# krullgit/3D-Object-Detection-for-autonomous-navigation

Measured on AMD Instinct MI355X. Metric: frames/sec (whole node) + p50 per-frame ms, 16k-pt pillars, higher is better.
Workload: dtype f32 (GEMMs on the 16-bit matrix pipe as split operands -- two float16 pieces per value, 3 products, fp32 accumulate: fp32-equivalent results, measured 1.5e-6 max from the fp32 oracle at this shape)

## Files before the change

3d-object-detection-for-autonomous-navigation_amd/csrc/backbone.hip:

```cpp
#include <stdio.h>
#include <stdlib.h>
#include <string.h>

#include "pp_common.h"

typedef float f32x16 __attribute__((ext_vector_type(16)));
#if PP_SPLIT_MODE == 0
typedef __bf16 bf16x8 __attribute__((ext_vector_type(8)));
#define PC_MFMA(A, B, C) __builtin_amdgcn_mfma_f32_32x32x16_bf16(A, B, C, 0, 0, 0)
#else
typedef _Float16 bf16x8 __attribute__((ext_vector_type(8)));
#define PC_MFMA(A, B, C) __builtin_amdgcn_mfma_f32_32x32x16_f16(A, B, C, 0, 0, 0)
#endif
#if PP_SPLIT_MODE == 0
#define PC_LO(PTR) (*reinterpret_cast<const bf16x8*>(PTR))
#else
#define PC_LO(PTR) (bf16x8{})
#endif
#if PP_SPLIT_MODE == 0
#define PC_PRODUCTS(ACC, XH, XM, XL, YH, YM, YL) \
    ACC = PC_MFMA(XL, YH, ACC); ACC = PC_MFMA(XH, YL, ACC); ACC = PC_MFMA(XM, YM, ACC); \
    ACC = PC_MFMA(XM, YH, ACC); ACC = PC_MFMA(XH, YM, ACC); ACC = PC_MFMA(XH, YH, ACC);
#elif PP_SPLIT_MODE == 1
#define PC_PRODUCTS(ACC, XH, XM, XL, YH, YM, YL) \
    ACC = PC_MFMA(XM, YH, ACC); ACC = PC_MFMA(XH, YM, ACC); ACC = PC_MFMA(XH, YH, ACC);
#else
#define PC_PRODUCTS(ACC, XH, XM, XL, YH, YM, YL) \
    ACC = PC_MFMA(XM, YM, ACC); ACC = PC_MFMA(XM, YH, ACC); ACC = PC_MFMA(XH, YM, ACC); ACC = PC_MFMA(XH, YH, ACC);
#endif
typedef unsigned u32x4 __attribute__((ext_vector_type(4)));

__device__ __forceinline__ float4 buf_load16(__amdgpu_buffer_rsrc_t r, unsigned voff, unsigned soff) {
    const u32x4 v = __builtin_amdgcn_raw_buffer_load_b128(r, voff, soff, 0);
    return make_float4(__uint_as_float(v.x), __uint_as_float(v.y), __uint_as_float(v.z), __uint_as_float(v.w));
}
__device__ __forceinline__ void buf_store16(float4 v, __amdgpu_buffer_rsrc_t r, unsigned voff, unsigned soff) {
    const u32x4 u = {__float_as_uint(v.x), __float_as_uint(v.y), __float_as_uint(v.z), __float_as_uint(v.w)};
    __builtin_amdgcn_raw_buffer_store_b128(u, r, voff, soff, 0);
}
__device__ __forceinline__ __amdgpu_buffer_rsrc_t make_rsrc(const void* base) {
    return __builtin_amdgcn_make_buffer_rsrc(const_cast<void*>(base), 0, 0x7ffffffe, 0x00020000);
}

#define PX_TILE 128

int g_num_cus = 256;

static bool split_precision() {
    static int dflt = -1;
    if (dflt < 0) {
        const char* e = getenv("PP_GEMM_PREC");
        dflt = (e && e[0] == 'f') ? 0 : 1;
    }
    return dflt == 1;
}
#define KC 32
#define LDS_STRIDE 36

struct GemmArgs {
    const float* in;
    const float* dw;
    const float* wt;
    const unsigned short* wt16;
    int n_total;
    const float* bias;
    float* out;
    float* head;
    const float* head_wt;
    const float* head_wt16;
    const float* head_bias;
    int head_mode;
    int M;
    int tile_lo;
    int in_h, in_w, cin;
    int px_h, px_w;
    int stride;
    int ld_out, co_off;
    int epi;
    int k, cout;
    const int* occ;
    int occ_nz;
    const unsigned long long* occbits;
    int occ_w64;
    float* cls_plane;
    int cls_col0, cls_ncol;
// ... 509 lines not shown
        const f16x2_t m = __builtin_convertvector(r1, f16x2_t);
        hi[j] = h.x; hi[j + 1] = h.y;
        mid[j] = m.x; mid[j + 1] = m.y;
    }
    lo = mid;
}
#endif

__device__ __forceinline__ void fast_divmod(int n, int d, float inv_d, int& q, int& r) {
    q = (int)((float)n * inv_d);
    r = n - q * d;
    if (r < 0) { --q; r += d; }
    if (r >= d) { ++q; r -= d; }
}

template <int NT, int S, int WPS, int PREC, int OCC = 0, int TR = 0>
__global__ __launch_bounds__(256, WPS) void k_sep_u(GemmArgs a, int ntiles) {
    static_assert(TR == 0 || (PREC == 1 && OCC == 0), "training forward: split-precision, dense input");
    constexpr bool PW = TR == 2;
    constexpr int NTAP = (TR == 1) ? 11 : 9;
    constexpr int KCH = 16, LSTR = KCH + 4, G = 4;
    constexpr int WW = S + 3;
    constexpr int NLD = PW ? 2 : 3 * WW;
    constexpr int SAW = 32 * LSTR;
    constexpr int SB = (PREC == 0) ? NT * LSTR : PP_NPIECE * NT * 8;
    constexpr int NB4 = (PREC == 0) ? (NT * G + 255) / 256 : (NT * 2 * PP_NPIECE + 255) / 256;
    constexpr int NTILES = NT / 32;
    constexpr int KQ = KCH / 8;
    __shared__ __attribute__((aligned(16))) float smem[8 * SAW + 2 * SB + (PW ? 0 : NTAP * 256) + (TR ? 8 * NT : 0)];
    const int tid = threadIdx.x, lane = tid & 63, wave = tid >> 6;
    float* const sAw = smem + wave * 2 * SAW;
    float* const sB = smem + 8 * SAW;
    float* const sDW = smem + 8 * SAW + 2 * SB;
    [[maybe_unused]] float* const sST = smem + 8 * SAW + 2 * SB + (PW ? 0 : NTAP * 256);

    const int xcd = blockIdx.x & 7, gl = blockIdx.x >> 3, GL = gridDim.x >> 3;
    const int nt_ = ntiles - a.tile_lo;
    const int tbase = a.tile_lo + (int)(((long long)xcd * nt_) >> 3), tend = a.tile_lo + (int)(((long long)(xcd + 1) * nt_) >> 3);
    const int first = tbase + gl;
    const int n0 = blockIdx.y * NT;
    if (first >= tend) {
        if (TR && a.tr_stat != nullptr && tid < 2 * NT)
            a.tr_stat[((size_t)blockIdx.x * 2 + tid / NT) * a.n_total + n0 + tid % NT] = 0.f;
        if (TR && a.tr_stat != nullptr && tid == 0 && blockIdx.y == 0) a.tr_stat[(size_t)gridDim.x * 2 * a.n_total + blockIdx.x] = 0.f;
        return;
    }
    const int ntl = (tend - first + GL - 1) / GL;
    const int cin = a.cin;
    const int nchunks = cin / KCH;
// ... 67 lines not shown
            aoff[e] = (ok_ ? rowoff_[dy_] + coloff_[dx_] : 0u) + (unsigned)(c4 * 16);                    \
        }                                                                                                \
        }                                                                                                \
    }
    constexpr int NBI = (PREC == 0) ? NT * G : NT * 2 * PP_NPIECE;
    unsigned boff[NB4];
    int bdst[NB4];
#pragma unroll
    for (int r = 0; r < NB4; ++r) {
        const int e_ = (tid + 256 * r) % NBI;
        if (PREC == 0) {
            boff[r] = (unsigned)(((n0 + e_ / G) * cin + (e_ % G) * 4) * 4);
            bdst[r] = (e_ / G) * LSTR + (e_ % G) * 4;
        } else {
            const int piece = e_ / (NT * 2), rem = e_ % (NT * 2), row = rem >> 1, half = rem & 1;
            boff[r] = (unsigned)(((piece * a.n_total + n0 + row) * 16 + half * 8) * 2);
            bdst[r] = piece * (NT * 8) + row * 8 + ((half ^ ((row >> 3) & 1)) * 4);
        }
    }
    const unsigned bstep = (PREC == 0) ? (unsigned)(KCH * 4) : (unsigned)(PP_NPIECE * a.n_total * 32);
    float4 rin[NLD];
    float4 rb0, rb1, rb2;
    rb0 = rb1 = rb2 = make_float4(0.f, 0.f, 0.f, 0.f);
    static_assert(NB4 <= 3, "weight prefetch registers");
#define U_LOAD_ACT(KCIDX, RIN)                                                                           \
    {                                                                                                    \
        const unsigned so_ = (unsigned)(KCIDX) * (KCH * 4);                                              \
        _Pragma("unroll") for (int e = 0; e < NLD; ++e) RIN[e] = buf_load16(rs_in, aoff[e], so_);        \
    }
#define U_LOAD_WT(KCIDX)                                                                                 \
    {                                                                                                    \
        const unsigned sb_ = (unsigned)(KCIDX) * bstep;                                                  \
// ... 4 lines not shown
#define U_LOAD_CHUNK(KCIDX) { U_LOAD_ACT(KCIDX, rin) U_LOAD_WT(KCIDX) }
    int ld_tile = first, ld_kc = 0;
    int st_kc = 0;
    int mm_tile = first, mm_kc = 0;
    [[maybe_unused]] float st_n = 0.f;
    U_TILE_OFFSETS(ld_tile)
    U_LOAD_CHUNK(0)
    ld_kc = 1;
    {
        const int ngrp = cin / 4;
        if (!PW) for (int e = tid; e < 9 * ngrp; e += 256) {
            const int t = e / ngrp, g4 = e - t * ngrp;
            reinterpret_cast<float4*>(sDW)[g4 * NTAP + t] = reinterpret_cast<const float4*>(a.dw)[e];
        }
        if (TR) for (int e = tid; e < 8 * NT; e += 256) sST[e] = 0.f;
        if (tr_act) {
            for (int g4 = tid; g4 < ngrp; g4 += 256) {
                const float4 q0 = a.tr_coef[4 * g4], q1 = a.tr_coef[4 * g4 + 1], q2 = a.tr_coef[4 * g4 + 2], q3 = a.tr_coef[4 * g4 + 3];
                reinterpret_cast<float4*>(sDW)[g4 * NTAP + 9] = make_float4(q0.x, q1.x, q2.x, q3.x);
                reinterpret_cast<float4*>(sDW)[g4 * NTAP + 10] = make_float4(q0.y, q1.y, q2.y, q3.y);
            }
        }
    }

    f32x16 acc[NTILES];
#pragma unroll
    for (int n = 0; n < NTILES; ++n)
#pragma unroll
        for (int r = 0; r < 16; ++r) acc[n][r] = 0.f;
    const int h = lane >> 5, r32 = lane & 31;
    float bias_r[NTILES];
#pragma unroll
    for (int n = 0; n < NTILES; ++n) bias_r[n] = (TR && a.bias == nullptr) ? 0.f : a.bias[n0 + n * 32 + r32];
    __syncthreads();

#define U_MFMA(I)                                                                                        \
    if (PREC == 1) {                                                                                     \
        const float* cA = cA0 + ((I) & 1) * SAW;                                                         \
        const float* cB = cB0 + ((I) & 1) * SB;                                                          \
        const float4 a0 = *reinterpret_cast<const float4*>(cA), a1 = *reinterpret_cast<const float4*>(cA + 4);  \
        const float av[8] = {a0.x, a0.y, a0.z, a0.w, a1.x, a1.y, a1.z, a1.w};                            \
        bf16x8 ah, am, al;                                                                               \
        split_bf16x3(av, ah, am, al);                                                                    \
        _Pragma("unroll") for (int n = 0; n < NTILES; ++n) {                                             \
            const bf16x8 bh = *reinterpret_cast<const bf16x8*>(cB + n * 32 * 8);                         \
            const bf16x8 bm = *reinterpret_cast<const bf16x8*>(cB + NT * 8 + n * 32 * 8);                \
            [[maybe_unused]] const bf16x8 bl = PC_LO(cB + 2 * NT * 8 + n * 32 * 8);            \
            PC_PRODUCTS(acc[n], ah, am, al, bh, bm, bl)                                                  \
        }                                                                                                \
    }                                                                                                    \
    if (PREC == 0) {                                                                                     \
        const float* cA = sAw + ((I) & 1) * SAW + r32 * LSTR + h * (KCH / 2);                            \
        const float* cB = sB + ((I) & 1) * SB + r32 * LSTR + h * (KCH / 2);                              \
        float4 a4[KQ];                                                                                   \
        _Pragma("unroll") for (int qq = 0; qq < KQ; ++qq) a4[qq] = *reinterpret_cast<const float4*>(cA + qq * 4);  \
        _Pragma("unroll") for (int n = 0; n < NTILES; ++n) {                                             \
            float4 b4[KQ];                                                                               \
            _Pragma("unroll") for (int qq = 0; qq < KQ; ++qq) b4[qq] = *reinterpret_cast<const float4*>(cB + n * 32 * LSTR + qq * 4);  \
            _Pragma("unroll") for (int qq = 0; qq < KQ; ++qq) {                                          \
                acc[n] = __builtin_amdgcn_mfma_f32_32x32x2f32(a4[qq].x, b4[qq].x, acc[n], 0, 0, 0);      \
                acc[n] = __builtin_amdgcn_mfma_f32_32x32x2f32(a4[qq].y, b4[qq].y, acc[n], 0, 0, 0);      \
                acc[n] = __builtin_amdgcn_mfma_f32_32x32x2f32(a4[qq].z, b4[qq].z, acc[n], 0, 0, 0);      \
                acc[n] = __builtin_amdgcn_mfma_f32_32x32x2f32(a4[qq].w, b4[qq].w, acc[n], 0, 0, 0);      \
// ... 21 lines not shown
                    o0.x = fmaf(v0.x, w4.x, o0.x); o0.y = fmaf(v0.y, w4.y, o0.y);                        \
                    o0.z = fmaf(v0.z, w4.z, o0.z); o0.w = fmaf(v0.w, w4.w, o0.w);                        \
                    o1.x = fmaf(v1.x, w4.x, o1.x); o1.y = fmaf(v1.y, w4.y, o1.y);                        \
                    o1.z = fmaf(v1.z, w4.z, o1.z); o1.w = fmaf(v1.w, w4.w, o1.w);                        \
                }                                                                                        \
        }                                                                                                \
        float* dA = sAw + buf * SAW + (2 * q) * LSTR + c4 * 4;                                           \
        *reinterpret_cast<float4*>(dA) = o0;                                                             \
        *reinterpret_cast<float4*>(dA + LSTR) = o1;                                                      \
        if (d_out) {        \
                                                                               \
            const unsigned dv_ = doff + (unsigned)st_kc * (KCH * 4);                                     \
            buf_store16(o0, rs_d, dv_, 0u);                                                              \
            buf_store16(o1, rs_d, dv_ + (unsigned)cin4, 0u);                                             \
        }                                                                                                \
        if (NBI % 256 == 0 || NB4 > 1 || tid < NBI) *reinterpret_cast<float4*>(sB + buf * SB + bdst[0]) = rb0;  \
        if (NB4 > 1 && (NBI >= 512 || tid + 256 < NBI)) *reinterpret_cast<float4*>(sB + buf * SB + bdst[NB4 > 1 ? 1 : 0]) = rb1;  \
        if (NB4 > 2 && (NBI >= 768 || tid + 512 < NBI)) *reinterpret_cast<float4*>(sB + buf * SB + bdst[NB4 > 2 ? 2 : 0]) = rb2;  \
        twp += 4 * (4 * NTAP);                                                                           \
        if (++st_kc == nchunks) { st_kc = 0; twp = sDW + c4 * (4 * NTAP); }                              \
    }
#define U_STAGE(P) U_STAGE2(P, rin)
#define U_ISSUE()                                                                                        \
    {                                                                                                    \
        if (ld_kc == 0) U_TILE_OFFSETS(ld_tile)                                                          \
        U_LOAD_CHUNK(ld_kc)                                                                              \
        if (++ld_kc == nchunks) { ld_kc = 0; ld_tile += GL; }                                            \
    }
#define U_ACT(X) (TR ? (X) : relu_keep_nan(X))
#define U_EPILOGUE()                                                                                     \
    {                                                                                                    \
        const int pw = mm_tile * 128 + wave * 32;                                                        \
        [[maybe_unused]] const int nw = min(max(a.M - pw, 0), 32);    \
// ... 46 lines not shown
                }                                                                                        \
            }                                                                                            \
        }                                                                                                \
        _Pragma("unroll") for (int n = 0; n < NTILES; ++n)                                               \
            _Pragma("unroll") for (int r = 0; r < 16; ++r) acc[n][r] = 0.f;                              \
        mm_kc = 0;                                                                                       \
        mm_tile += GL;                                                                                   \
    }

    const float* twp = sDW + c4 * (4 * NTAP);
    const float* const cA0 = sAw + r32 * LSTR + h * (KCH / 2);
    const float* const cB0 = sB + r32 * 8 + ((h ^ ((r32 >> 3) & 1)) * 4);
    U_STAGE(0)
    U_ISSUE()
    __syncthreads();
    int i = 0;
    for (; i + 3 < total; i += 2) {
        U_MFMA(0)
        U_STAGE(1)
        U_ISSUE()
        if (++mm_kc == nchunks) U_EPILOGUE()
        __syncthreads();
        U_MFMA(1)
        U_STAGE(0)
        U_ISSUE()
        if (++mm_kc == nchunks) U_EPILOGUE()
        __syncthreads();
    }
    U_MFMA(0)
    U_STAGE(1)
// ... 5 lines not shown
    if (TR && a.tr_stat != nullptr) {
        __syncthreads();
        const float* red = sST;
        float wn[4] = {0.f, 0.f, 0.f, 0.f};
        for (int t = first; t < tend; t += GL)
#pragma unroll
            for (int w = 0; w < 4; ++w) wn[w] += (float)min(max(a.M - (t * 128 + w * 32), 0), 32);
        if (tid < NT) {
            float n_ = 0.f, s_ = 0.f, m_ = 0.f;
#pragma unroll
            for (int w = 0; w < 4; ++w) bn_chan_merge(n_, s_, m_, wn[w], red[(w * 2) * NT + tid], red[(w * 2 + 1) * NT + tid]);
            a.tr_stat[((size_t)blockIdx.x * 2 + 0) * a.n_total + n0 + tid] = s_;
            a.tr_stat[((size_t)blockIdx.x * 2 + 1) * a.n_total + n0 + tid] = m_;
        }
        if (tid == 0 && blockIdx.y == 0) a.tr_stat[(size_t)gridDim.x * 2 * a.n_total + blockIdx.x] = ((wn[0] + wn[1]) + wn[2]) + wn[3];
    }
#undef U_MFMA
#undef U_STAGE
#undef U_ISSUE
#undef U_EPILOGUE
#undef U_ACT
#undef U_LOAD_CHUNK
#undef U_TILE_OFFSETS
}

template <int NT, int S, int WPS, int WPB>
static void launch_u(const GemmArgs& a, int n_total, hipStream_t s) {
    const int ntiles = (a.M + 127) / 128;
    const int ny = n_total / NT;
    const bool bf = a.wt16 != nullptr && split_precision();
// ... 457 lines not shown
    return 2 * ((M + 31) / 32 * (n_total / 64)) <= (long long)half_cus * g_num_cus;
}
static bool sep_k8_runs(int cin, int n_total, long long M) {
    return cin % 256 == 0 && (M + 31) / 32 * (n_total / 64) <= (long long)g_num_cus;
}
template <int S>
static void launch_k4(const GemmArgs& a, int n_total, hipStream_t s) {
    dim3 grid((unsigned)((a.M + 31) / 32), n_total / 64);
    if (sep_k8_runs(a.cin, n_total, a.M)) {
        PP_LAUNCH("k_sep_k4", (k_sep_k4<64, S, 8>), grid, dim3(512), 0, s, a);
        return;
    }
    PP_LAUNCH("k_sep_k4", (k_sep_k4<64, S>), grid, dim3(256), 0, s, a);
}

#define DCH(R, H) (((R) & 3) + 8 * ((R) >> 2) + 4 * (H))
template <int NT>
__device__ __forceinline__ void deconv_tile_epilogue(const GemmArgs& a, f32x16 (&acc)[NT / 32],
                                                     int tile, int wave, int lane, int cbase, int delta,
                                                     const int* opix_tab, const float* sHW, const float* s_hbias) {
    constexpr int NTILES = NT / 32;
    const int h = lane >> 5, r32 = lane & 31;
    const int pix = tile * 128 + wave * 32 + r32;
    if (tile * 128 + wave * 32 >= a.M) return;
    const bool ok = pix < a.M;
    const size_t orow = (size_t)(opix_tab[wave * 32 + r32] + delta);
    const bool heads = a.head_mode != 0;
    float* hrow = a.head + orow * PP_HEAD_COLS + 4 * h;
    f32x16 hacc;
    if (a.head_mode == 2 && ok) {
#pragma unroll
// ... 659 lines not shown
}

template <int NT>
static void launch_deconv_u(const GemmArgs& a, int n_total, hipStream_t s) {
    constexpr int WPS = 3;
    const int ntiles = (a.M + 127) / 128;
    const int ny = n_total / NT;
    int slots = (g_num_cus * WPS) / ny;
    if (slots < 8) slots = 8;
    int gx = ntiles < slots ? ntiles : slots;
    gx = (gx + 7) & ~7;
    dim3 grid((unsigned)gx, ny);
    PP_LAUNCH("k_deconv_u", (k_deconv_u<NT, WPS>), grid, dim3(256), 0, s, a, ntiles);
}

template <int NT, int MODE>
static void launch_t(const GemmArgs& a, int n_total, hipStream_t s) {
    const unsigned mt = (unsigned)((a.M + PX_TILE - 1) / PX_TILE);
    dim3 grid(mt, n_total / NT);
    PP_LAUNCH("k_gemm_layer", (k_gemm_layer<NT, MODE>), grid, dim3(256), 0, s, a);
}

static bool ws_small_tile(long long M, int n_total, int NT) {
    const long long tiles128 = ((M + 127) / 128) * (n_total / NT);
    return tiles128 < 256;
}

template <int NT, int MODE, int S>
static void launch_ws(const GemmArgs& a, int n_total, hipStream_t s) {
    if (ws_small_tile(a.M, n_total, NT)) {
// ... 44 lines not shown
}

bool sparse_input_supported(const LayerDesc& L, int batch) {
    return L.kind == LAYER_SEP && use_ws(L) && sep_uniform() && L.d_wt16 != nullptr && split_precision() &&
           (long long)batch * L.out_h * L.out_w < (1 << 24);
}

bool deconv_can_fuse_heads(const LayerDesc& L) {
    return L.kind == LAYER_DECONV && (L.cout == 32 || L.cout == 64 || L.cout == 128) && use_ws(L);
}

static long long layer_rows(const LayerDesc& L, int batch) {
    return (L.kind == LAYER_SEP) ? (long long)batch * L.out_h * L.out_w : (long long)batch * L.in_h * L.in_w;
}

std::string layer_kernel_name(const LayerDesc& L, int batch) {
    const int nt = (L.kind == LAYER_HEAD) ? 32 : (L.cout % 128 == 0 ? 128 : (L.cout % 64 == 0 ? 64 : 32));
    const int mode = (L.kind == LAYER_SEP) ? 0 : 1;
    char buf[64];
    if (L.kind == LAYER_SEP && use_ws(L) && sep_uniform() && layer_rows(L, batch) < (1 << 24)) {
        if (sep_k4_runs(L.d_wt16, L.cin, L.n_total, layer_rows(L, batch))) {
            if (sep_k8_runs(L.cin, L.n_total, layer_rows(L, batch))) snprintf(buf, sizeof(buf), "k_sep_k4<64,%d,8>", L.stride);
            else snprintf(buf, sizeof(buf), "k_sep_k4<64,%d>", L.stride);
            return std::string(buf);
        }
        if (sep_p_runs(L.d_wt16, L.stride, L.cin, L.cout, L.n_total, layer_rows(L, batch), L.d_occ)) return std::string("k_sep_p");
        const int unt = sep_u_nt(L, batch);
        const bool bf = L.d_wt16 != nullptr && split_precision();
        int wps;
        if (L.stride == 1) wps = bf ? (unt == 128 ? PP_SEP128_WPB : (unt == 64 ? PP_SEP64_WPB : 3)) : (unt == 128 ? 3 : 4);
        else wps = bf ? (unt == 128 ? 2 : 3) : (unt == 128 ? 2 : (unt == 64 ? 3 : 4));
// ... 1 lines not shown
    } else if (deconv_uniform(L) && deconv_k4_runs(L, layer_rows(L, batch))) {
        snprintf(buf, sizeof(buf), "k_deconv_k4<%d>", nt);
    } else if (deconv_uniform(L) && deconv_r_runs(L)) {
        snprintf(buf, sizeof(buf), "k_deconv_r<%d>", L.cin);
    } else if (deconv_uniform(L)) {
        snprintf(buf, sizeof(buf), "k_deconv_u<%d,3>", nt);
    } else if (use_ws(L)) {
        const int pxb = ws_small_tile(layer_rows(L, batch), L.n_total, nt) ? 64 : 128;
        snprintf(buf, sizeof(buf), "k_gemm_ws<%d,%d,%d,%d>", nt, mode, mode == 0 ? L.stride : 1, pxb);
    } else {
        snprintf(buf, sizeof(buf), "k_gemm_layer<%d,%d>", nt, mode);
    }
    return std::string(buf);
}

bool layer_writes_cls_plane(const LayerDesc& L) {
    return L.kind == LAYER_DECONV && L.head_mode == 2 && L.d_cls_plane != nullptr && deconv_uniform(L);
}

bool launch_layer_subrange_ok(const LayerDesc& L, int frame0, int batch, int total_batch) {
    if (L.kind != LAYER_SEP) return false;
    const long long hw = (long long)L.out_h * L.out_w;
    if ((frame0 * hw) % PX_TILE != 0) return false;
    return layer_kernel_name(L, batch).compare(0, 8, "k_sep_u<") == 0 && layer_kernel_name(L, total_batch).compare(0, 8, "k_sep_u<") == 0;
}

int launch_layer(const LayerDesc& L, int batch, float* d_head, hipStream_t s, int frame0) {
    if (batch <= 0) return 0;
    if (L.cin % KC != 0) return PP_ERR_UNSUPPORTED;
    {
        const long long m_sep = (long long)batch * L.out_h * L.out_w, m_in = (long long)batch * L.in_h * L.in_w;
        if (m_sep >= (1ll << 31) - PX_TILE || m_in >= (1ll << 31) - PX_TILE ||
            (long long)batch * L.out_h * L.out_w * L.k * L.k >= (1ll << 31)) return PP_ERR_UNSUPPORTED;
    }
    GemmArgs a;
    a.tile_lo = 0;
    a.in = L.in; a.dw = L.d_dw; a.wt = L.d_wt; a.bias = L.d_bias; a.out = L.out;
    a.wt16 = reinterpret_cast<const unsigned short*>(L.d_wt16); a.n_total = L.n_total;
    a.head = d_head; a.head_wt = L.d_head_wt; a.head_bias = L.d_head_bias; a.head_mode = L.head_mode;
    a.head_wt16 = L.d_head_wt16;
    a.in_h = L.in_h; a.in_w = L.in_w; a.cin = L.cin;
    a.stride = L.stride; a.ld_out = L.ld_out; a.co_off = L.co_off;
    a.k = L.k; a.cout = L.cout;
    a.occ = L.d_occ; a.occ_nz = L.occ_nz;
    a.occbits = L.d_occbits; a.occ_w64 = occ_words(L.in_w);
    a.tr_coef = nullptr; a.tr_D = nullptr; a.tr_stat = nullptr;
    a.cls_plane = layer_writes_cls_plane(L) ? L.d_cls_plane : nullptr;
    a.cls_col0 = L.cls_col0; a.cls_ncol = L.cls_ncol;
    if (L.kind == LAYER_SEP) {
        a.px_h = L.out_h; a.px_w = L.out_w; a.epi = 0;
        a.M = (frame0 + batch) * L.out_h * L.out_w;
        if (frame0 > 0) {
            if (!launch_layer_subrange_ok(L, frame0, batch, frame0 + batch)) return PP_ERR_UNSUPPORTED;
            a.tile_lo = (int)(((long long)frame0 * L.out_h * L.out_w) / PX_TILE);
        }
        if (L.cout % 32 != 0) return PP_ERR_UNSUPPORTED;
        if (a.occ != nullptr && !sparse_input_supported(L, batch))
            return PP_ERR_UNSUPPORTED;
        if (use_ws(L) && sep_uniform() && a.M < (1 << 24)) {
            const int nt = sep_u_nt(L, batch);
            const long long msel = (long long)batch * L.out_h * L.out_w;
#if PP_SPLIT_MODE != 0
            if (!sep_k4_runs(a.wt16, a.cin, L.n_total, msel) &&
                sep_p_runs(a.wt16, L.stride, a.cin, L.cout, L.n_total, msel, a.occ)) {
                launch_p(a, s);
            } else
#endif
            if (sep_k4_runs(a.wt16, a.cin, L.n_total, msel)) {
                if (L.stride == 1) launch_k4<1>(a, L.n_total, s);
                else launch_k4<2>(a, L.n_total, s);
            } else if (L.stride == 1) {
// ... 60 lines not shown
```

3d-object-detection-for-autonomous-navigation_amd/csrc/pp_api.hip:

```cpp
#include <math.h>
#include <cmath>
#include <algorithm>
#include <functional>
#include <mutex>
#include <stdarg.h>
#include <stdio.h>
#include <stdlib.h>
#include <string.h>
#include <unordered_map>

#include "pp_common.h"
#include "train.h"

extern int g_num_cus;

namespace {

std::string g_create_error;

struct KTime { const char* name; int ev; };

}

thread_local PpProf g_pp_prof = {nullptr, nullptr};
// ... 442 lines not shown
    if (e->occbits_live && e->nz == 1) {
        launch_anchor_mask_bits(e->d_occbits, batch, e->ny, e->nx, e->d_cells, e->A, e->cfg.anchor_area_threshold, e->d_mask,
                                e->stream);
        HIPCHK(e, hipGetLastError());
        return PP_OK;
    }
    launch_anchor_mask(e->d_cellmap, batch, e->nz, e->ny, e->nx, e->d_cells, e->A, e->cfg.anchor_area_threshold,
                       e->d_integ, e->d_mask, e->stream);
    HIPCHK(e, hipGetLastError());
    return PP_OK;
}

void refresh_tags(pp_engine* e, int batch) {
    if (e->tag_batch == batch) return;
    for (size_t i = 0; i < e->layers.size(); ++i)
        e->layer_tags[i] = layer_kernel_name(e->layers[i], batch) + ":" + e->layers[i].name;
    e->tag_batch = batch;
}

int run_backbone(pp_engine* e, int batch) {
    refresh_tags(e, batch);
    e->cls_plane_live = false;
    for (const LayerDesc& L : e->layers) if (layer_writes_cls_plane(L)) e->cls_plane_live = true;
    const int sub_on = e->cache_budget_mb > 0 ? 1 : 0;
    const long sub_mb = e->cache_budget_mb;
    size_t i = 0;
    while (i < e->layers.size()) {
        size_t j = i;
        int sub = batch;
        if (sub_on && e->layers[i].kind == LAYER_SEP) {
            const LayerDesc& l0 = e->layers[i];
// ... 11 lines not shown
            }
            const double budget = (double)sub_mb * 1048576.0;
            while (sub > 1 && per_frame * sub > budget && sub % 2 == 0) sub /= 2;
            for (bool ok = false; sub < batch && !ok; ) {
                ok = true;
                for (size_t k = i; k < j && ok; ++k)
                    for (int f0 = 0; f0 < batch && ok; f0 += sub)
                        ok = launch_layer_subrange_ok(e->layers[k], f0, std::min(sub, batch - f0), batch) &&
                             (long long)sub * e->layers[k].out_h * e->layers[k].out_w >= 1024ll * 128;
                if (!ok) sub *= 2;
            }
            if (sub >= batch) sub = batch;
        } else {
            j = i + 1;
        }
        for (int f0 = 0; f0 < batch; f0 += sub) {
            const int nb = std::min(sub, batch - f0);
            for (size_t k = i; k < j; ++k) {
                LayerDesc L = e->layers[k];
                if (k == 0 && L.d_occ != nullptr) { L.d_occ = e->d_cellmap; L.d_occbits = e->occbits_live ? e->d_occbits : nullptr; }
                ProfScope ps(e, e->layer_tags[k].c_str());
                int st = launch_layer(L, nb, e->d_head, e->stream, f0);
                if (st) return fail(e, st, "layer %s: unsupported shape (cin=%d cout=%d)", L.name, L.cin, L.cout);
            }
        }
        i = j;
    }
    HIPCHK(e, hipGetLastError());
    return PP_OK;
}

int run_post(pp_engine* e, int batch, bool to_host = false) {
    PostParams p;
    p.batch = batch; p.A = e->A; p.pre_max = e->cfg.nms_pre_max_size; p.post_max = e->cfg.nms_post_max_size;
    p.score_thr = e->cfg.nms_score_threshold; p.iou_thr = e->cfg.nms_iou_threshold;
    p.head = e->d_head; p.cls = e->cls_plane_live ? e->d_cls : nullptr; p.napl = e->napl; p.ncls = e->ncls; p.use_dir = e->use_dir ? 1 : 0; p.mask = e->d_mask; p.anchors = e->d_anchors;
    p.calib = e->d_calib; p.dets = e->d_dets; p.n_dets = e->d_ndets;
    p.dets_host = to_host ? e->h_dets : nullptr; p.n_dets_host = to_host ? e->h_ndets : nullptr;
    ProfScope ps(e, "k_postprocess");
    launch_postprocess(p, e->stream);
    HIPCHK(e, hipGetLastError());
// ... 1684 lines not shown
```

3d-object-detection-for-autonomous-navigation_amd/csrc/pp_common.h:

```cpp
#pragma once

#include <hip/hip_runtime.h>
#include <stdint.h>

#include <map>
#include <string>
#include <vector>

#include <hip/hip_ext.h>

#include "../../include/pp_hip.h"

#define PP_WAVE 64
#ifndef PP_SPLIT_MODE
#define PP_SPLIT_MODE 1
#endif
#define PP_NPIECE ((PP_SPLIT_MODE == 0) ? 3 : 2)
#define PP_ZPAD_FLOATS 512
#define PP_HEAD_COLS 32

struct PpProf {
    pp_engine* e;
    const char* tag;
};
// ... 119 lines not shown
    uint8_t* am_mask;
};
bool pfn_can_carry_anchor_mask(const PfnParams& p, bool padded_source);
bool pfn_writes_occbits(const PfnParams& p, bool padded_source);
int launch_pfn(const PfnParams& p, bool padded_source, hipStream_t s);

void launch_anchor_mask(const int* cellmap, int batch, int nz, int ny, int nx, const int* cells, int64_t A,
                        float threshold, int* integ, uint8_t* mask, hipStream_t s);
__host__ __device__ static inline int occ_words(int nx) { return (nx + 2 + 63) / 64 + 1; }
void launch_anchor_mask_bits(const unsigned long long* occbits, int batch, int ny, int nx, const int* cells, int64_t A,
                             float threshold, uint8_t* mask, hipStream_t s);

bool deconv_can_fuse_heads(const LayerDesc& L);
bool layer_writes_cls_plane(const LayerDesc& L);
bool sparse_input_supported(const LayerDesc& L, int batch);
std::string layer_kernel_name(const LayerDesc& L, int batch);
struct SepTrainArgs {
    const float* in;
    const float4* coef;
    const float* dw;
    const unsigned short* wt16;
    float* Z;
    float* D;
    float* stat;
    int batch, in_h, in_w, cin, out_h, out_w, cout, stride;
    const char* tag;
};
int launch_sep_train(const SepTrainArgs& t, hipStream_t s);
struct RowsTrainArgs {
    const float* in;
    const unsigned short* wt16;
    const float* bias;
    float* out;
    float* stat;
    long long rows;
    int K, N, ld_out;
    const char* tag;
};
int launch_rows_train(const RowsTrainArgs& t, hipStream_t s);
int launch_layer(const LayerDesc& L, int batch, float* d_head, hipStream_t s, int frame0 = 0);
bool launch_layer_subrange_ok(const LayerDesc& L, int frame0, int batch, int total_batch);

struct PostParams {
    int batch;
    int64_t A;
    int pre_max, post_max;
    float score_thr, iou_thr;
    const float* head;
    const float* cls;
    int napl;
    int ncls;
    int use_dir;
    const uint8_t* mask;
    const float* anchors;
    const float* calib;
// ... 56 lines not shown
```

Before: 91130.

## Fuse stride-1 separable conv with following 1x1 deconv and head GEMM

Adds an FD variant of k_sep_u that, after computing a 64-channel separable conv tile, keeps the result in registers, splits it into f16 pieces and runs the following k=1 deconv (64->128) and the head projection inside the same kernel. Deconv and head weights are streamed in double-buffered LDS stages, and the layer loop skips the fused deconv layer. The intent is to avoid writing and re-reading the intermediate activation and to save a separate kernel launch. In exchange it uses more LDS and registers per block, which may lower occupancy, and it adds swapped-operand MFMA ordering and a row permutation of the weight layout.

```diff
diff --git a/3d-object-detection-for-autonomous-navigation_amd/csrc/backbone.hip b/3d-object-detection-for-autonomous-navigation_amd/csrc/backbone.hip
--- a/3d-object-detection-for-autonomous-navigation_amd/csrc/backbone.hip
+++ b/3d-object-detection-for-autonomous-navigation_amd/csrc/backbone.hip
@@ -28,6 +28,17 @@
 #define PC_PRODUCTS(ACC, XH, XM, XL, YH, YM, YL) \
     ACC = PC_MFMA(XM, YM, ACC); ACC = PC_MFMA(XM, YH, ACC); ACC = PC_MFMA(XH, YM, ACC); ACC = PC_MFMA(XH, YH, ACC);
 #endif
+#if PP_SPLIT_MODE == 0
+#define PC_PRODUCTS_SW(ACC, XH, XM, XL, YH, YM, YL) \
+    ACC = PC_MFMA(YH, XL, ACC); ACC = PC_MFMA(YL, XH, ACC); ACC = PC_MFMA(YM, XM, ACC); \
+    ACC = PC_MFMA(YH, XM, ACC); ACC = PC_MFMA(YM, XH, ACC); ACC = PC_MFMA(YH, XH, ACC);
+#elif PP_SPLIT_MODE == 1
+#define PC_PRODUCTS_SW(ACC, XH, XM, XL, YH, YM, YL) \
+    ACC = PC_MFMA(YH, XM, ACC); ACC = PC_MFMA(YM, XH, ACC); ACC = PC_MFMA(YH, XH, ACC);
+#else
+#define PC_PRODUCTS_SW(ACC, XH, XM, XL, YH, YM, YL) \
+    ACC = PC_MFMA(YM, XM, ACC); ACC = PC_MFMA(YH, XM, ACC); ACC = PC_MFMA(YM, XH, ACC); ACC = PC_MFMA(YH, XH, ACC);
+#endif
 typedef unsigned u32x4 __attribute__((ext_vector_type(4)));
 
 __device__ __forceinline__ float4 buf_load16(__amdgpu_buffer_rsrc_t r, unsigned voff, unsigned soff) {
@@ -43,6 +54,7 @@
 }
 
 #define PX_TILE 128
+#define DCH(R, H) (((R) & 3) + 8 * ((R) >> 2) + 4 * (H))
 
 int g_num_cus = 256;
 
@@ -69,6 +81,9 @@
     const float* head_wt;
     const float* head_wt16;
     const float* head_bias;
+    const unsigned short* fd_wt16;
+    const float* fd_bias;
+    int fd_n_total;
     int head_mode;
     int M;
     int tile_lo;
@@ -608,9 +623,10 @@
     if (r >= d) { ++q; r -= d; }
 }
 
-template <int NT, int S, int WPS, int PREC, int OCC = 0, int TR = 0>
+template <int NT, int S, int WPS, int PREC, int OCC = 0, int TR = 0, int FD = 0>
 __global__ __launch_bounds__(256, WPS) void k_sep_u(GemmArgs a, int ntiles) {
     static_assert(TR == 0 || (PREC == 1 && OCC == 0), "training forward: split-precision, dense input");
+    static_assert(FD == 0 || (NT == 64 && S == 1 && PREC == 1 && OCC == 0 && TR == 0 && PP_NPIECE == 2), "fused deconv");
     constexpr bool PW = TR == 2;
     constexpr int NTAP = (TR == 1) ? 11 : 9;
     constexpr int KCH = 16, LSTR = KCH + 4, G = 4;
@@ -621,12 +637,15 @@
     constexpr int NB4 = (PREC == 0) ? (NT * G + 255) / 256 : (NT * 2 * PP_NPIECE + 255) / 256;
     constexpr int NTILES = NT / 32;
     constexpr int KQ = KCH / 8;
-    __shared__ __attribute__((aligned(16))) float smem[8 * SAW + 2 * SB + (PW ? 0 : NTAP * 256) + (TR ? 8 * NT : 0)];
+    constexpr int SBF = FD ? 6 * PP_NPIECE * 256 : SB;
+    constexpr int NDW = PW ? 0 : NTAP * (FD ? 64 : 256);
+    __shared__ __attribute__((aligned(16))) float smem[8 * SAW + 2 * SBF + NDW + (TR ? 8 * NT : 0) + (FD ? 64 + 128 + 32 : 0)];
     const int tid = threadIdx.x, lane = tid & 63, wave = tid >> 6;
     float* const sAw = smem + wave * 2 * SAW;
     float* const sB = smem + 8 * SAW;
-    float* const sDW = smem + 8 * SAW + 2 * SB;
-    [[maybe_unused]] float* const sST = smem + 8 * SAW + 2 * SB + (PW ? 0 : NTAP * 256);
+    float* const sDW = smem + 8 * SAW + 2 * SBF;
+    [[maybe_unused]] float* const sST = smem + 8 * SAW + 2 * SBF + NDW;
+    [[maybe_unused]] float* const sFB = smem + 8 * SAW + 2 * SBF + NDW;
 
     const int xcd = blockIdx.x & 7, gl = blockIdx.x >> 3, GL = gridDim.x >> 3;
     const int nt_ = ntiles - a.tile_lo;
@@ -724,8 +743,9 @@
             bdst[r] = (e_ / G) * LSTR + (e_ % G) * 4;
         } else {
             const int piece = e_ / (NT * 2), rem = e_ % (NT * 2), row = rem >> 1, half = rem & 1;
+            const int prow = FD ? ((row & ~12) | ((row & 4) << 1) | ((row & 8) >> 1)) : row;
             boff[r] = (unsigned)(((piece * a.n_total + n0 + row) * 16 + half * 8) * 2);
-            bdst[r] = piece * (NT * 8) + row * 8 + ((half ^ ((row >> 3) & 1)) * 4);
+            bdst[r] = piece * (NT * 8) + prow * 8 + ((half ^ ((prow >> 3) & 1)) * 4);
         }
     }
     const unsigned bstep = (PREC == 0) ? (unsigned)(KCH * 4) : (unsigned)(PP_NPIECE * a.n_total * 32);
@@ -760,6 +780,11 @@
             reinterpret_cast<float4*>(sDW)[g4 * NTAP + t] = reinterpret_cast<const float4*>(a.dw)[e];
         }
         if (TR) for (int e = tid; e < 8 * NT; e += 256) sST[e] = 0.f;
+        if (FD) {
+            if (tid < 64) sFB[tid] = a.bias[tid];
+            if (tid < 128) sFB[64 + tid] = a.fd_bias[tid];
+            if (tid < PP_HEAD_COLS) sFB[192 + tid] = a.head_bias[tid];
+        }
         if (tr_act) {
             for (int g4 = tid; g4 < ngrp; g4 += 256) {
                 const float4 q0 = a.tr_coef[4 * g4], q1 = a.tr_coef[4 * g4 + 1], q2 = a.tr_coef[4 * g4 + 2], q3 = a.tr_coef[4 * g4 + 3];
@@ -783,7 +808,7 @@
 #define U_MFMA(I)                                                                                        \
     if (PREC == 1) {                                                                                     \
         const float* cA = cA0 + ((I) & 1) * SAW;                                                         \
-        const float* cB = cB0 + ((I) & 1) * SB;                                                          \
+        const float* cB = cB0 + ((I) & 1) * SBF;                                                         \
         const float4 a0 = *reinterpret_cast<const float4*>(cA), a1 = *reinterpret_cast<const float4*>(cA + 4);  \
         const float av[8] = {a0.x, a0.y, a0.z, a0.w, a1.x, a1.y, a1.z, a1.w};                            \
         bf16x8 ah, am, al;                                                                               \
@@ -792,7 +817,8 @@
             const bf16x8 bh = *reinterpret_cast<const bf16x8*>(cB + n * 32 * 8);                         \
             const bf16x8 bm = *reinterpret_cast<const bf16x8*>(cB + NT * 8 + n * 32 * 8);                \
             [[maybe_unused]] const bf16x8 bl = PC_LO(cB + 2 * NT * 8 + n * 32 * 8);            \
-            PC_PRODUCTS(acc[n], ah, am, al, bh, bm, bl)                                                  \
+            if (FD) { PC_PRODUCTS_SW(acc[n], ah, am, al, bh, bm, bl) }                                   \
+            else { PC_PRODUCTS(acc[n], ah, am, al, bh, bm, bl) }                                         \
         }                                                                                                \
     }                                                                                                    \
     if (PREC == 0) {                                                                                     \
@@ -844,9 +870,9 @@
             buf_store16(o0, rs_d, dv_, 0u);                                                              \
             buf_store16(o1, rs_d, dv_ + (unsigned)cin4, 0u);                                             \
         }                                                                                                \
-        if (NBI % 256 == 0 || NB4 > 1 || tid < NBI) *reinterpret_cast<float4*>(sB + buf * SB + bdst[0]) = rb0;  \
-        if (NB4 > 1 && (NBI >= 512 || tid + 256 < NBI)) *reinterpret_cast<float4*>(sB + buf * SB + bdst[NB4 > 1 ? 1 : 0]) = rb1;  \
-        if (NB4 > 2 && (NBI >= 768 || tid + 512 < NBI)) *reinterpret_cast<float4*>(sB + buf * SB + bdst[NB4 > 2 ? 2 : 0]) = rb2;  \
+        if (NBI % 256 == 0 || NB4 > 1 || tid < NBI) *reinterpret_cast<float4*>(sB + buf * SBF + bdst[0]) = rb0;  \
+        if (NB4 > 1 && (NBI >= 512 || tid + 256 < NBI)) *reinterpret_cast<float4*>(sB + buf * SBF + bdst[NB4 > 1 ? 1 : 0]) = rb1;  \
+        if (NB4 > 2 && (NBI >= 768 || tid + 512 < NBI)) *reinterpret_cast<float4*>(sB + buf * SBF + bdst[NB4 > 2 ? 2 : 0]) = rb2;  \
         twp += 4 * (4 * NTAP);                                                                           \
         if (++st_kc == nchunks) { st_kc = 0; twp = sDW + c4 * (4 * NTAP); }                              \
     }
@@ -923,6 +949,131 @@
     U_STAGE(0)
     U_ISSUE()
     __syncthreads();
+    if constexpr (FD) {
+    static_assert(PP_HEAD_COLS == 32, "head row = one 32-column MFMA tile");
+    const __amdgpu_buffer_rsrc_t rs_fw = make_rsrc(a.fd_wt16), rs_fh = make_rsrc(a.head_wt16);
+    const int fd_n_total = a.fd_n_total;
+#define FD_FOFF(R) ((unsigned)(((((tid + 256 * (R)) >> 7) * PP_NPIECE + ((tid >> 6) & 1)) * fd_n_total + ((tid >> 1) & 31)) * 32 + (tid & 1) * 16))
+#define FD_FDST(R) (((tid + 256 * (R)) >> 7) * (PP_NPIECE * 256) + ((tid >> 6) & 1) * 256 + ((tid >> 1) & 31) * 8 + (((tid & 1) ^ ((tid >> 4) & 1)) * 4))
+#define FD_LOAD_E(ND)                                                                                    \
+    {                                                                                                    \
+        rb0 = buf_load16(rs_fw, FD_FOFF(0), (unsigned)(ND) * 1024u);                                     \
+        rb1 = buf_load16(rs_fw, FD_FOFF(1), (unsigned)(ND) * 1024u);                                     \
+        rb2 = buf_load16(rs_fh, (unsigned)tid * 16u, (unsigned)(ND) * 4096u);                            \
+    }
+#define FD_STAGE_E(BUF)                                                                                  \
+    {                                                                                                    \
+        *reinterpret_cast<float4*>(sB + (BUF) * SBF + FD_FDST(0)) = rb0;                                 \
+        *reinterpret_cast<float4*>(sB + (BUF) * SBF + FD_FDST(1)) = rb1;                                 \
+              \
+        *reinterpret_cast<float4*>(sB + (BUF) * SBF + 4 * PP_NPIECE * 256 + ((tid ^ ((tid >> 4) & 1)) * 4)) = rb2;  \
+    }
+    bf16x8 xh[4], xm[4], xl[4];
+    f32x16 hacc;
+#define FD_EPILOGUE13()                                                                                  \
+    {                                                                                                    \
+        const int pw = mm_tile * 128 + wave * 32;                                                        \
+        const int qi = lane & 3, qb = r32 >> 2;                                                          \
+        const unsigned dst = (unsigned)((pw + 4 * qb) * a.ld_out + a.co_off + n0 + 16 * (qi >> 1) + 8 * h + 4 * (qi & 1)) * 4u;  \
+        _Pragma("unroll") for (int n = 0; n < 2; ++n) {      \
+            _Pragma("unroll") for (int u = 0; u < 4; ++u) {                                              \
+                const float4 b4 = *reinterpret_cast<const float4*>(sFB + n * 32 + 16 * (u >> 1) + 8 * h + 4 * (u & 1));  \
+                acc[n][4 * u + 0] = relu_keep_nan(acc[n][4 * u + 0] + b4.x);                             \
+                acc[n][4 * u + 1] = relu_keep_nan(acc[n][4 * u + 1] + b4.y);                             \
+                acc[n][4 * u + 2] = relu_keep_nan(acc[n][4 * u + 2] + b4.z);                             \
+                acc[n][4 * u + 3] = relu_keep_nan(acc[n][4 * u + 3] + b4.w);                             \
+            }                                                                                            \
+            if (pw < a.M) {                                                                              \
+                float t[4][4];                                                               \
+                _Pragma("unroll") for (int j = 0; j < 4; ++j) {                                          \
+                    float x0 = acc[n][j], x1 = acc[n][4 + j], x2 = acc[n][8 + j], x3 = acc[n][12 + j];   \
+                    quad_transpose4(x0, x1, x2, x3, lane);                                               \
+                    t[0][j] = x0; t[1][j] = x1; t[2][j] = x2; t[3][j] = x3;                              \
+                }                                                                                        \
+                _Pragma("unroll") for (int u = 0; u < 4; ++u)                                            \
+                    if (pw + 4 * qb + u < a.M)                                                           \
+                        buf_store16(make_float4(t[u][0], t[u][1], t[u][2], t[u][3]), rs_out,             \
+                                    dst + (unsigned)((u * a.ld_out + n * 32) * 4), 0u);                  \
+            }                                                                                            \
+            _Pragma("unroll") for (int c = 2 * n; c < 2 * n + 2; ++c) {                                  \
+                const float av[8] = {acc[n][8 * (c & 1) + 0], acc[n][8 * (c & 1) + 1], acc[n][8 * (c & 1) + 2],  \
+                                     acc[n][8 * (c & 1) + 3], acc[n][8 * (c & 1) + 4], acc[n][8 * (c & 1) + 5],  \
+                                     acc[n][8 * (c & 1) + 6], acc[n][8 * (c & 1) + 7]};                  \
+                split_bf16x3(av, xh[c], xm[c], xl[c]);                                                   \
+            }                                                                                            \
+        }                                                                                                \
+    }
+    bf16x8 yh[2], ym[2], yl[2];
+#define FD_MFMA_D(ND, BUF)                                                                               \
+    {                                                                                                    \
+        const float* cE_ = sB + (BUF) * SBF + r32 * 8 + ((h ^ ((r32 >> 3) & 1)) * 4);                    \
+        f32x16 dacc_;                                                                                    \
+        _Pragma("unroll") for (int r = 0; r < 16; ++r) dacc_[r] = sFB[64 + (ND) * 32 + DCH(r, h)];        \
+        if ((ND) == 0) { _Pragma("unroll") for (int r = 0; r < 16; ++r) hacc[r] = sFB[192 + DCH(r, h)]; } \
+        _Pragma("unroll") for (int c = 0; c < 4; ++c) {                                                  \
+            const bf16x8 wh_ = *reinterpret_cast<const bf16x8*>(cE_ + c * (PP_NPIECE * 256));            \
+            const bf16x8 wm_ = *reinterpret_cast<const bf16x8*>(cE_ + c * (PP_NPIECE * 256) + 256);      \
+            [[maybe_unused]] const bf16x8 wl_ = PC_LO(cE_ + c * (PP_NPIECE * 256) + 512);                \
+            PC_PRODUCTS(dacc_, wh_, wm_, wl_, xh[c], xm[c], xl[c])                                       \
+        }                                                                                                \
+        _Pragma("unroll") for (int g = 0; g < 2; ++g) {                                                  \
+            const float av[8] = {relu_keep_nan(dacc_[8 * g + 0]), relu_keep_nan(dacc_[8 * g + 1]),      \
+                                 relu_keep_nan(dacc_[8 * g + 2]), relu_keep_nan(dacc_[8 * g + 3]),      \
+                                 relu_keep_nan(dacc_[8 * g + 4]), relu_keep_nan(dacc_[8 * g + 5]),      \
+                                 relu_keep_nan(dacc_[8 * g + 6]), relu_keep_nan(dacc_[8 * g + 7])};     \
+            split_bf16x3(av, yh[g], ym[g], yl[g]);                                                       \
+        }                                                                                                \
+    }
+#define FD_MFMA_H(BUF)                                                                                   \
+    {                                                                                                    \
+        const float* cE_ = sB + (BUF) * SBF + r32 * 8 + ((h ^ ((r32 >> 3) & 1)) * 4);                    \
+        _Pragma("unroll") for (int g = 0; g < 2; ++g) {                                                  \
+            const float* hW_ = cE_ + 4 * PP_NPIECE * 256 + g * (PP_NPIECE * 256);                        \
+            const bf16x8 hh_ = *reinterpret_cast<const bf16x8*>(hW_);                                    \
+            const bf16x8 hm_ = *reinterpret_cast<const bf16x8*>(hW_ + 256);                              \
+            [[maybe_unused]] const bf16x8 hl_ = PC_LO(hW_ + 512);                                        \
+            PC_PRODUCTS(hacc, hh_, hm_, hl_, yh[g], ym[g], yl[g])                                        \
+        }                                                                                                \
+    }
+#define FD_MFMA_E(ND, BUF) FD_MFMA_D(ND, BUF) FD_MFMA_H(BUF)
+    const __amdgpu_buffer_rsrc_t rs_out = make_rsrc(a.out), rs_head = make_rsrc(a.head);
+    for (mm_tile = first; mm_tile < tend; mm_tile += GL) {
+        const bool more = mm_tile + GL < tend;
+#pragma unroll
+        for (int n = 0; n < NTILES; ++n)
+#pragma unroll
+            for (int r = 0; r < 16; ++r) acc[n][r] = 0.f;
+        U_MFMA(0) U_STAGE(1) U_LOAD_CHUNK(2) __syncthreads();
+        U_MFMA(1) U_STAGE(0) U_LOAD_CHUNK(3) __syncthreads();
+        U_MFMA(0) U_STAGE(1) FD_LOAD_E(0) __syncthreads();
+        U_MFMA(1) FD_STAGE_E(0) FD_EPILOGUE13() FD_LOAD_E(1) __syncthreads();
+        FD_MFMA_E(0, 0) FD_STAGE_E(1) FD_LOAD_E(2) __syncthreads();
+        FD_MFMA_E(1, 1) FD_STAGE_E(0) FD_LOAD_E(3) __syncthreads();
+        FD_MFMA_E(2, 0) FD_STAGE_E(1)
+        if (more) { U_TILE_OFFSETS(mm_tile + GL) U_LOAD_CHUNK(0) }
+        __syncthreads();
+        FD_MFMA_E(3, 1)
+        {
+            const int pix = mm_tile * 128 + wave * 32 + r32;
+            if (pix < a.M) {
+                const unsigned hrow = (unsigned)(pix * PP_HEAD_COLS + 4 * h) * 4u;
+#pragma unroll
+                for (int g = 0; g < 4; ++g)
+                    buf_store16(make_float4(hacc[4 * g], hacc[4 * g + 1], hacc[4 * g + 2], hacc[4 * g + 3]), rs_head, hrow + 32u * g, 0u);
+            }
+        }
+        if (more) { U_STAGE(0) U_LOAD_CHUNK(1) }
+        __syncthreads();
+    }
+#undef FD_MFMA_E
+#undef FD_MFMA_H
+#undef FD_MFMA_D
+#undef FD_EPILOGUE13
+#undef FD_STAGE_E
+#undef FD_LOAD_E
+#undef FD_FDST
+#undef FD_FOFF
+    } else {
     int i = 0;
     for (; i + 3 < total; i += 2) {
         U_MFMA(0)
@@ -958,6 +1109,7 @@
             a.tr_stat[((size_t)blockIdx.x * 2 + 1) * a.n_total + n0 + tid] = m_;
         }
         if (tid == 0 && blockIdx.y == 0) a.tr_stat[(size_t)gridDim.x * 2 * a.n_total + blockIdx.x] = ((wn[0] + wn[1]) + wn[2]) + wn[3];
+    }
     }
 #undef U_MFMA
 #undef U_STAGE
@@ -1445,7 +1597,6 @@
     PP_LAUNCH("k_sep_k4", (k_sep_k4<64, S>), grid, dim3(256), 0, s, a);
 }
 
-#define DCH(R, H) (((R) & 3) + 8 * ((R) >> 2) + 4 * (H))
 template <int NT>
 __device__ __forceinline__ void deconv_tile_epilogue(const GemmArgs& a, f32x16 (&acc)[NT / 32],
                                                      int tile, int wave, int lane, int cbase, int delta,
@@ -2135,6 +2286,17 @@
     PP_LAUNCH("k_deconv_u", (k_deconv_u<NT, WPS>), grid, dim3(256), 0, s, a, ntiles);
 }
 
+#if PP_SPLIT_MODE != 0
+static void launch_u_fd(const GemmArgs& a, hipStream_t s) {
+    const int ntiles = (a.M + 127) / 128;
+    const int slots = g_num_cus * 3;
+    const int mine = ntiles - a.tile_lo;
+    int gx = mine < slots ? mine : slots;
+    gx = (gx + 7) & ~7;
+    PP_LAUNCH("k_sep_u", (k_sep_u<64, 1, 3, 1, 0, 0, 1>), dim3((unsigned)gx, 1), dim3(256), 0, s, a, ntiles);
+}
+#endif
+
 template <int NT, int MODE>
 static void launch_t(const GemmArgs& a, int n_total, hipStream_t s) {
     const unsigned mt = (unsigned)((a.M + PX_TILE - 1) / PX_TILE);
@@ -2209,7 +2371,8 @@
     return (L.kind == LAYER_SEP) ? (long long)batch * L.out_h * L.out_w : (long long)batch * L.in_h * L.in_w;
 }
 
-std::string layer_kernel_name(const LayerDesc& L, int batch) {
+std::string layer_kernel_name(const LayerDesc& L, int batch, const LayerDesc* next) {
+    if (next != nullptr && sep_fuses_deconv(L, *next, batch)) return std::string("k_sep_u<64,1,3,1,0,0,1>");
     const int nt = (L.kind == LAYER_HEAD) ? 32 : (L.cout % 128 == 0 ? 128 : (L.cout % 64 == 0 ? 64 : 32));
     const int mode = (L.kind == LAYER_SEP) ? 0 : 1;
     char buf[64];
@@ -2241,6 +2404,32 @@
     return std::string(buf);
 }
 
+[[maybe_unused]] static bool fd_shape_ok(const LayerDesc& L, const LayerDesc& D) {
+    if (L.kind != LAYER_SEP || L.stride != 1 || L.cin != 64 || L.cout != 64 || L.n_total != 64 || L.d_wt16 == nullptr ||
+        L.d_occ != nullptr || L.out == nullptr || L.ld_out % 4 != 0)
+        return false;
+    if (D.kind != LAYER_DECONV || D.k != 1 || D.cin != 64 || D.cout != 128 || D.n_total != 128 || D.head_mode != 1 ||
+        D.d_wt16 == nullptr || D.d_head_wt16 == nullptr || D.out != nullptr || D.in != L.out || D.in_h != L.out_h ||
+        D.in_w != L.out_w)
+        return false;
+    return true;
+}
+bool sep_fuses_deconv(const LayerDesc& L, const LayerDesc& D, int batch) {
+#if PP_SPLIT_MODE == 0
+    (void)L; (void)D; (void)batch;
+    return false;
+#else
+    static int on = -1;
+    if (on < 0) { const char* e = getenv("PP_FUSE_DECONV"); on = (e && e[0] == '0') ? 0 : 1; }
+    if (!on || !split_precision() || !fd_shape_ok(L, D)) return false;
+    const long long rows = (long long)batch * L.out_h * L.out_w;
+    if (rows * L.ld_out * 4 >= (1ll << 31) - 4096) return false;
+    if (!deconv_uniform(D) || deconv_k4_runs(D, rows) || deconv_r_runs(D)) return false;
+    const std::string k = layer_kernel_name(L, batch);
+    return k.compare(0, 12, "k_sep_u<64,1") == 0;
+#endif
+}
+
 bool layer_writes_cls_plane(const LayerDesc& L) {
     return L.kind == LAYER_DECONV && L.head_mode == 2 && L.d_cls_plane != nullptr && deconv_uniform(L);
 }
@@ -2252,7 +2441,7 @@
     return layer_kernel_name(L, batch).compare(0, 8, "k_sep_u<") == 0 && layer_kernel_name(L, total_batch).compare(0, 8, "k_sep_u<") == 0;
 }
 
-int launch_layer(const LayerDesc& L, int batch, float* d_head, hipStream_t s, int frame0) {
+int launch_layer(const LayerDesc& L, int batch, float* d_head, hipStream_t s, int frame0, const LayerDesc* fuse) {
     if (batch <= 0) return 0;
     if (L.cin % KC != 0) return PP_ERR_UNSUPPORTED;
     {
@@ -2274,6 +2463,7 @@
     a.tr_coef = nullptr; a.tr_D = nullptr; a.tr_stat = nullptr;
     a.cls_plane = layer_writes_cls_plane(L) ? L.d_cls_plane : nullptr;
     a.cls_col0 = L.cls_col0; a.cls_ncol = L.cls_ncol;
+    a.fd_wt16 = nullptr; a.fd_bias = nullptr; a.fd_n_total = 0;
     if (L.kind == LAYER_SEP) {
         a.px_h = L.out_h; a.px_w = L.out_w; a.epi = 0;
         a.M = (frame0 + batch) * L.out_h * L.out_w;
@@ -2282,6 +2472,23 @@
             a.tile_lo = (int)(((long long)frame0 * L.out_h * L.out_w) / PX_TILE);
         }
         if (L.cout % 32 != 0) return PP_ERR_UNSUPPORTED;
+        if (fuse != nullptr) {
+#if PP_SPLIT_MODE != 0
+            if (!split_precision() || !fd_shape_ok(L, *fuse) || a.M >= (1 << 24) ||
+                layer_kernel_name(L, batch).compare(0, 12, "k_sep_u<64,1") != 0)
+                return PP_ERR_UNSUPPORTED;
+            a.fd_wt16 = reinterpret_cast<const unsigned short*>(fuse->d_wt16);
+            a.fd_bias = fuse->d_bias;
+            a.fd_n_total = fuse->n_total;
+            a.head_wt16 = fuse->d_head_wt16;
+            a.head_bias = fuse->d_head_bias;
+            a.head_mode = 1;
+            launch_u_fd(a, s);
+            return 0;
+#else
+            return PP_ERR_UNSUPPORTED;
+#endif
+        }
         if (a.occ != nullptr && !sparse_input_supported(L, batch))
             return PP_ERR_UNSUPPORTED;
         if (use_ws(L) && sep_uniform() && a.M < (1 << 24)) {
diff --git a/3d-object-detection-for-autonomous-navigation_amd/csrc/pp_api.hip b/3d-object-detection-for-autonomous-navigation_amd/csrc/pp_api.hip
--- a/3d-object-detection-for-autonomous-navigation_amd/csrc/pp_api.hip
+++ b/3d-object-detection-for-autonomous-navigation_amd/csrc/pp_api.hip
@@ -480,7 +480,8 @@
 void refresh_tags(pp_engine* e, int batch) {
     if (e->tag_batch == batch) return;
     for (size_t i = 0; i < e->layers.size(); ++i)
-        e->layer_tags[i] = layer_kernel_name(e->layers[i], batch) + ":" + e->layers[i].name;
+        e->layer_tags[i] = layer_kernel_name(e->layers[i], batch, i + 1 < e->layers.size() ? &e->layers[i + 1] : nullptr) +
+                           ":" + e->layers[i].name;
     e->tag_batch = batch;
 }
 
@@ -522,17 +523,18 @@
         } else {
             j = i + 1;
         }
+        const LayerDesc* fused = (j < e->layers.size() && sep_fuses_deconv(e->layers[j - 1], e->layers[j], batch)) ? &e->layers[j] : nullptr;
         for (int f0 = 0; f0 < batch; f0 += sub) {
             const int nb = std::min(sub, batch - f0);
             for (size_t k = i; k < j; ++k) {
                 LayerDesc L = e->layers[k];
                 if (k == 0 && L.d_occ != nullptr) { L.d_occ = e->d_cellmap; L.d_occbits = e->occbits_live ? e->d_occbits : nullptr; }
                 ProfScope ps(e, e->layer_tags[k].c_str());
-                int st = launch_layer(L, nb, e->d_head, e->stream, f0);
+                int st = launch_layer(L, nb, e->d_head, e->stream, f0, k + 1 == j ? fused : nullptr);
                 if (st) return fail(e, st, "layer %s: unsupported shape (cin=%d cout=%d)", L.name, L.cin, L.cout);
             }
         }
-        i = j;
+        i = fused != nullptr ? j + 1 : j;
     }
     HIPCHK(e, hipGetLastError());
     return PP_OK;
diff --git a/3d-object-detection-for-autonomous-navigation_amd/csrc/pp_common.h b/3d-object-detection-for-autonomous-navigation_amd/csrc/pp_common.h
--- a/3d-object-detection-for-autonomous-navigation_amd/csrc/pp_common.h
+++ b/3d-object-detection-for-autonomous-navigation_amd/csrc/pp_common.h
@@ -157,7 +157,8 @@
 bool deconv_can_fuse_heads(const LayerDesc& L);
 bool layer_writes_cls_plane(const LayerDesc& L);
 bool sparse_input_supported(const LayerDesc& L, int batch);
-std::string layer_kernel_name(const LayerDesc& L, int batch);
+std::string layer_kernel_name(const LayerDesc& L, int batch, const LayerDesc* next = nullptr);
+bool sep_fuses_deconv(const LayerDesc& L, const LayerDesc& D, int batch);
 struct SepTrainArgs {
     const float* in;
     const float4* coef;
@@ -181,7 +182,7 @@
     const char* tag;
 };
 int launch_rows_train(const RowsTrainArgs& t, hipStream_t s);
-int launch_layer(const LayerDesc& L, int batch, float* d_head, hipStream_t s, int frame0 = 0);
+int launch_layer(const LayerDesc& L, int batch, float* d_head, hipStream_t s, int frame0 = 0, const LayerDesc* fuse = nullptr);
 bool launch_layer_subrange_ok(const LayerDesc& L, int frame0, int batch, int total_batch);
 
 struct PostParams {
```

Result: no change. 90100 (median of 2 runs) (-1.1%).
